# francescofugazzi/3dgsconverter

Measured on NVIDIA H100. Metric: Msplats/s SOR k=16, higher is better.
Workload: dtype f32

## Files before the change

### 3dgsconverter_b200/csrc/gsx_radix.cu

```cuda
#include "../../include/gsx.h"

#include "gsx_common.cuh"
#include "gsx_radix.cuh"

namespace gsx {

#define GSX_FULL 0xffffffffu
constexpr int kRsThreads = 256;
constexpr int kRsPerThread = 16;
constexpr int kRsTile = kRsThreads * kRsPerThread;
constexpr int kRsWarpKeys = 32 * kRsPerThread;
constexpr int kScanBlock = 2048;

__global__ void __launch_bounds__(256) k_scan_block(uint32_t* __restrict__ data, int64_t n,
                                                    uint32_t* __restrict__ sums) {
    const int64_t base = (int64_t)blockIdx.x * kScanBlock + (int64_t)threadIdx.x * 8;
    uint32_t v[8];
    uint32_t tsum = 0;
#pragma unroll
    for (int e = 0; e < 8; ++e) {
        v[e] = base + e < n ? data[base + e] : 0u;
        tsum += v[e];
    }
    uint32_t x = tsum;
// ... 134 lines not shown
        }
        __shared__ uint32_t wtot[8];
        if (lane == 31) wtot[w] = x;
        __syncthreads();
        uint32_t woff = 0;
#pragma unroll
        for (int i = 0; i < 8; ++i)
            if (i < w) woff += wtot[i];
        dstart[threadIdx.x] = woff + x - dcount;
    }
    __syncthreads();
#pragma unroll
    for (int e = 0; e < kRsPerThread; ++e) {
        const int64_t i = wbase + e * 32 + lane;
        if (i < n) {
            const uint32_t d = (uint32_t)(key[e] >> shift) & dmask;
            const uint32_t lp = dstart[d] + wcnt[w][d] + rank[e];
            skeys[lp] = key[e];
            svals[lp] = vals_in[i];
        }
    }
    __syncthreads();
    const int cnt = (int)(n - tbase < kRsTile ? n - tbase : kRsTile);
    for (int j = threadIdx.x; j < cnt; j += kRsThreads) {
        const uint64_t k = skeys[j];
        const uint32_t d = (uint32_t)(k >> shift) & dmask;
        const uint32_t pos = gbase[d] + ((uint32_t)j - dstart[d]);
        keys_out[pos] = k;
        vals_out[pos] = svals[j];
    }
}

constexpr uint32_t kOsAgg = 1u << 30, kOsInc = 1u << 31, kOsVal = (1u << 30) - 1u;
constexpr int kOsMaxPass = 8;
constexpr uint32_t kOsSpinLimit = 1u << 22;

__global__ void __launch_bounds__(256) k_os_hist(const uint64_t* __restrict__ keys, int64_t n, int begin_bit,
                                                  int npass, uint32_t last_mask, uint32_t* __restrict__ ghist) {
    __shared__ uint32_t sh[kOsMaxPass * 256];
    for (int t = threadIdx.x; t < npass * 256; t += 256) sh[t] = 0;
    __syncthreads();
    const int64_t stride = (int64_t)gridDim.x * 256;
    for (int64_t i = (int64_t)blockIdx.x * 256 + threadIdx.x; i < n; i += stride) {
        const uint64_t k = keys[i] >> begin_bit;
        for (int p = 0; p < npass; ++p)
            atomicAdd(&sh[p * 256 + ((uint32_t)(k >> (8 * p)) & (p == npass - 1 ? last_mask : 255u))], 1u);
    }
    __syncthreads();
    for (int t = threadIdx.x; t < npass * 256; t += 256)
        if (sh[t]) atomicAdd(&ghist[t], sh[t]);
}

__global__ void __launch_bounds__(256) k_os_scan(uint32_t* __restrict__ ghist) {
    uint32_t* h = ghist + blockIdx.x * 256;
    const int lane = threadIdx.x & 31, w = threadIdx.x >> 5;
    const uint32_t v = h[threadIdx.x];
    uint32_t x = v;
#pragma unroll
    for (int o = 1; o < 32; o <<= 1) {
        uint32_t y = __shfl_up_sync(GSX_FULL, x, o);
        if (lane >= o) x += y;
    }
    __shared__ uint32_t wt[8];
    if (lane == 31) wt[w] = x;
    __syncthreads();
    uint32_t woff = 0;
#pragma unroll
    for (int i = 0; i < 8; ++i)
        if (i < w) woff += wt[i];
    h[threadIdx.x] = woff + x - v;
}

template <bool PAIRS>
constexpr size_t os_pass_smem() {
    return (size_t)kRsTile * (PAIRS ? 12 : 8) + (size_t)8 * 256 * 4 + 2 * 256 * 4;
}

template <bool PAIRS>
__global__ void __launch_bounds__(kRsThreads, PAIRS ? 3 : 4)
    k_os_pass(const uint64_t* __restrict__ keys_in, const int32_t* __restrict__ vals_in, uint64_t* __restrict__ keys_out,
              int32_t* __restrict__ vals_out, int64_t n, int shift, uint32_t dmask, const uint32_t* __restrict__ gbase_pass,
              uint32_t* lookback, unsigned int* tile_counter) {
// ... 71 lines not shown
        uint32_t woff = 0;
#pragma unroll
        for (int i = 0; i < 8; ++i)
            if (i < w) woff += wtot[i];
        dstart[threadIdx.x] = woff + x - dcount;
    }
    __syncthreads();
#pragma unroll
    for (int e = 0; e < kRsPerThread; ++e) {
        const int64_t i = wbase + e * 32 + lane;
        if (i < n) {
            const uint32_t d = (uint32_t)(key[e] >> shift) & dmask;
            const uint32_t lp = dstart[d] + wcnt[w][d] + ((rank2[e >> 1] >> (16 * (e & 1))) & 0xffffu);
            skeys[lp] = key[e];
            if (PAIRS) svals[lp] = vals_in[i];
        }
    }
    __syncthreads();
    const int cnt = (int)(n - tbase < kRsTile ? n - tbase : kRsTile);
    for (int j = threadIdx.x; j < cnt; j += kRsThreads) {
        const uint64_t k = skeys[j];
        const uint32_t d = (uint32_t)(k >> shift) & dmask;
        const uint32_t pos = gbase[d] + ((uint32_t)j - dstart[d]);
        keys_out[pos] = k;
        if (PAIRS) vals_out[pos] = svals[j];
    }
}

static size_t os_ws_elems(int64_t n) {
    const int64_t ntiles = (n + kRsTile - 1) / kRsTile;
    return (size_t)kOsMaxPass * 256 + 64 + (size_t)kOsMaxPass * 256 * ntiles;
}

template <bool PAIRS>
static int onesweep_sort(uint64_t* keys0, uint64_t* keys1, int32_t* vals0, int32_t* vals1, int64_t n, int begin_bit,
                         int end_bit, uint32_t* ws, uint64_t** keys_sorted, int32_t** vals_sorted, cudaStream_t st) {
    const int64_t ntiles = (n + kRsTile - 1) / kRsTile;
    const int npass = (end_bit - begin_bit + 7) / 8;
    uint32_t* ghist = ws;
    unsigned int* counters = ws + kOsMaxPass * 256;
    uint32_t* lookback = ws + kOsMaxPass * 256 + 64;
    GSX_CUDA_CHECK(cudaMemsetAsync(ws, 0, ((size_t)kOsMaxPass * 256 + 64 + (size_t)npass * 256 * ntiles) * sizeof(uint32_t), st));
    static int hist_blocks = 0;
    if (!hist_blocks) {
        int dev = 0, sms = 132;
        cudaGetDevice(&dev);
        cudaDeviceGetAttribute(&sms, cudaDevAttrMultiProcessorCount, dev);
        hist_blocks = sms * 8;
    }
    int64_t hb = (n + 255) / 256;
    if (hb > hist_blocks) hb = hist_blocks;
    const uint32_t last_mask = digit_mask(begin_bit + 8 * (npass - 1), end_bit);
    k_os_hist<<<(unsigned)hb, 256, 0, st>>>(keys0, n, begin_bit, npass, last_mask, ghist);
    GSX_KERNEL_CHECK();
    k_os_scan<<<npass, 256, 0, st>>>(ghist);
    GSX_KERNEL_CHECK();
    GSX_CUDA_CHECK(cudaFuncSetAttribute(k_os_pass<PAIRS>, cudaFuncAttributeMaxDynamicSharedMemorySize, (int)os_pass_smem<PAIRS>()));
    uint64_t *kin = keys0, *kout = keys1;
    int32_t *vin = vals0, *vout = vals1;
    for (int p = 0; p < npass; ++p) {
        k_os_pass<PAIRS><<<(unsigned)ntiles, kRsThreads, os_pass_smem<PAIRS>(), st>>>(
            kin, vin, kout, vout, n, begin_bit + 8 * p, p == npass - 1 ? last_mask : 255u, ghist + p * 256,
            lookback + (size_t)p * 256 * ntiles, counters + p);
        GSX_KERNEL_CHECK();
        uint64_t* tk = kin;
        kin = kout;
        kout = tk;
        int32_t* tv = vin;
        vin = vout;
        vout = tv;
    }
    *keys_sorted = kin;
    if (vals_sorted) *vals_sorted = vin;
    return GSX_OK;
}

size_t radix_ws_bytes(int64_t n) {
    if (n < 1) n = 1;
    int64_t ntiles = (n + kRsTile - 1) / kRsTile;
    size_t hist = (size_t)256 * ntiles;
    size_t three_kernel = hist + scan_ws_elems((int64_t)hist) + 256;
    size_t onesweep = os_ws_elems(n);
    return (three_kernel > onesweep ? three_kernel : onesweep) * sizeof(uint32_t);
}

int radix_sort_pairs(uint64_t* keys0, uint64_t* keys1, int32_t* vals0, int32_t* vals1, int64_t n, int begin_bit,
                     int end_bit, void* ws, size_t ws_bytes, uint64_t** keys_sorted, int32_t** vals_sorted,
                     cudaStream_t st) {
    GSX_NVTX("gsx::radix_sort_pairs");
    GSX_REQUIRE(n >= 1 && n < 4294967296ll, GSX_ERR_ARG, "radix: n out of range");
    GSX_REQUIRE(ws_bytes >= radix_ws_bytes(n), GSX_ERR_WORKSPACE, "radix: workspace too small");
    GSX_REQUIRE(begin_bit >= 0 && end_bit <= 64 && begin_bit < end_bit, GSX_ERR_ARG, "radix: bad bit range");
    if (n < (1ll << 30))
        return onesweep_sort<true>(keys0, keys1, vals0, vals1, n, begin_bit, end_bit, (uint32_t*)ws, keys_sorted,
                                   vals_sorted, st);
    const int64_t ntiles = (n + kRsTile - 1) / kRsTile;
    uint32_t* hist = (uint32_t*)ws;
    uint32_t* scan_ws = hist + (size_t)256 * ntiles;
    GSX_CUDA_CHECK(cudaFuncSetAttribute(k_rs_scatter, cudaFuncAttributeMaxDynamicSharedMemorySize, (int)kRsScatterSmem));
    uint64_t *kin = keys0, *kout = keys1;
    int32_t *vin = vals0, *vout = vals1;
    for (int shift = begin_bit; shift < end_bit; shift += 8) {
        const uint32_t dmask = digit_mask(shift, end_bit);
        k_rs_hist<<<(unsigned)ntiles, kRsThreads, 0, st>>>(kin, n, shift, dmask, ntiles, hist);
        GSX_KERNEL_CHECK();
        int rc = exclusive_scan_u32(hist, (int64_t)256 * ntiles, scan_ws, st);
        if (rc) return rc;
        k_rs_scatter<<<(unsigned)ntiles, kRsThreads, kRsScatterSmem, st>>>(kin, vin, kout, vout, n, shift, dmask, ntiles,
                                                                          hist);
        GSX_KERNEL_CHECK();
        uint64_t* tk = kin;
        kin = kout;
        kout = tk;
        int32_t* tv = vin;
        vin = vout;
        vout = tv;
    }
    *keys_sorted = kin;
    *vals_sorted = vin;
    return GSX_OK;
}

int radix_sort_keys(uint64_t* keys0, uint64_t* keys1, int64_t n, int begin_bit, int end_bit, void* ws, size_t ws_bytes,
                    uint64_t** keys_sorted, cudaStream_t st) {
    GSX_NVTX("gsx::radix_sort_keys");
    GSX_REQUIRE(n >= 1 && n < (1ll << 30), GSX_ERR_ARG, "radix: n out of range");
    GSX_REQUIRE(ws_bytes >= radix_ws_bytes(n), GSX_ERR_WORKSPACE, "radix: workspace too small");
    GSX_REQUIRE(begin_bit >= 0 && end_bit <= 64 && begin_bit < end_bit, GSX_ERR_ARG, "radix: bad bit range");
    return onesweep_sort<false>(keys0, keys1, nullptr, nullptr, n, begin_bit, end_bit, (uint32_t*)ws, keys_sorted, nullptr,
                                st);
}

}

using namespace gsx;

extern "C" {

int64_t gsx_sort_pairs_workspace_bytes(int64_t n) {
    if (n < 1) n = 1;
    return (int64_t)(align_up((size_t)n * 8, 256) + align_up((size_t)n * 4, 256) + radix_ws_bytes(n) + 1024);
}

int gsx_sort_pairs(uint64_t* keys_dev, int32_t* vals_dev, int64_t n, int32_t begin_bit, int32_t end_bit, void* ws,
                   int64_t ws_bytes, void* stream) {
    cudaStream_t st = (cudaStream_t)stream;
    if (n == 0) return GSX_OK;
    GSX_REQUIRE(ws_bytes >= gsx_sort_pairs_workspace_bytes(n), GSX_ERR_WORKSPACE, "sort: workspace too small");
    Carver c(ws, (size_t)ws_bytes);
    uint64_t* k1 = c.take<uint64_t>((size_t)n);
    int32_t* v1 = c.take<int32_t>((size_t)n);
    char* rws = c.take<char>(radix_ws_bytes(n));
    uint64_t* ks = nullptr;
    int32_t* vs = nullptr;
    int rc = vals_dev ? radix_sort_pairs(keys_dev, k1, vals_dev, v1, n, begin_bit, end_bit, rws, radix_ws_bytes(n), &ks,
                                         &vs, st)
                      : radix_sort_keys(keys_dev, k1, n, begin_bit, end_bit, rws, radix_ws_bytes(n), &ks, st);
    if (rc) return rc;
    if (ks != keys_dev) {
        GSX_CUDA_CHECK(cudaMemcpyAsync(keys_dev, ks, (size_t)n * 8, cudaMemcpyDeviceToDevice, st));
        if (vals_dev) GSX_CUDA_CHECK(cudaMemcpyAsync(vals_dev, vs, (size_t)n * 4, cudaMemcpyDeviceToDevice, st));
    }
    return GSX_OK;
}

// ... 2 lines not shown
```

### 3dgsconverter_b200/csrc/gsx_radix.cuh

```cuda
#pragma once
#include "gsx_common.cuh"
namespace gsx {
size_t radix_ws_bytes(int64_t n);
size_t scan_workspace_bytes(int64_t n);
int exclusive_scan_u32_ws(uint32_t* data, int64_t n, uint32_t* ws, cudaStream_t st);
int radix_sort_pairs(uint64_t* keys0, uint64_t* keys1, int32_t* vals0, int32_t* vals1, int64_t n, int begin_bit,
                     int end_bit, void* ws, size_t ws_bytes, uint64_t** keys_sorted, int32_t** vals_sorted,
                     cudaStream_t st);
int radix_sort_keys(uint64_t* keys0, uint64_t* keys1, int64_t n, int begin_bit, int end_bit, void* ws, size_t ws_bytes,
                    uint64_t** keys_sorted, cudaStream_t st);
}
```

### 3dgsconverter_b200/csrc/gsx_sor.cu

```cuda
#include "../../include/gsx.h"

#include "gsx_bits.cuh"
#include "gsx_common.cuh"
#include "gsx_sor.cuh"

#include "gsx_radix.cuh"
#include <math.h>

namespace gsx {

#define GSX_D2LIM_BITS 0x60ad78ebu
#define GSX_FULL 0xffffffffu

constexpr int kCellCodeBits = 15;
constexpr float kCellCodeScale = (float)(1 << (kCellCodeBits / 3));
constexpr float kCellCodeMax = kCellCodeScale - 1.f;
constexpr int kSmallBucket = 64;
constexpr int kQueryBatch = 16;
constexpr int kMergeThreshold = 9;
constexpr int kKnnMinBlocks = 8;
constexpr int kFlatSupers = 8;
const char* sor_build_info() {
    return "knn=r03a;epi_smem=1;first_sort=1;query_batch=16;minblocks=8;merge_threshold=9;small_bucket=64;"
           "flat_supers=8;knn16=0;tma=0;i32=1;cell_order=hilbert15";
// ... 160 lines not shown

struct PackFmt {
    int idx_bits, mort_bits, bucket_bits;
    __host__ __device__ int key_shift() const { return idx_bits + mort_bits; }
    __host__ __device__ uint64_t idx_mask() const { return (1ull << idx_bits) - 1ull; }
    __host__ __device__ int sort_begin() const { return idx_bits; }
    __host__ __device__ int sort_end() const { return idx_bits + mort_bits + bucket_bits; }
};

static int bits_for(int64_t n) {
    int b = 1;
    while (((int64_t)1 << b) < n) ++b;
    return b;
}

static PackFmt pack_fmt(int64_t n_items, int64_t n_buckets) {
    PackFmt f;
    f.idx_bits = bits_for(n_items);
    f.bucket_bits = bits_for(n_buckets);
    int avail = 64 - f.idx_bits - f.bucket_bits;
    if (avail > kCellCodeBits) avail = kCellCodeBits;
    f.mort_bits = avail < 0 ? 0 : avail - avail % 3;
    return f;
}

__device__ __forceinline__ uint64_t pack_word(uint64_t key , uint64_t bucket_sub,
                                              int64_t idx, PackFmt f) {
    const uint64_t bucket = (key >> kCellCodeBits) - bucket_sub;
    const uint64_t mort = (key & ((1ull << kCellCodeBits) - 1ull)) >> (kCellCodeBits - f.mort_bits);
    return (((bucket << f.mort_bits) | mort) << f.idx_bits) | (uint64_t)idx;
}

__global__ void __launch_bounds__(256) k_sor_keys(const float* __restrict__ xyz, int64_t n, float bx, float by,
                                                  float bz, float cell, uint64_t M64, PackFmt f,
                                                  uint64_t* __restrict__ keys) {
    int64_t i = (int64_t)blockIdx.x * blockDim.x + threadIdx.x;
    if (i >= n) return;
    keys[i] = pack_word(bucket_key(xyz[3 * i], xyz[3 * i + 1], xyz[3 * i + 2], bx, by, bz, cell, n, M64), 0, i, f);
}

template <bool GATHER>
__device__ __forceinline__ void
    sor_finish_tile(const int64_t tile, const float* __restrict__ xyz, const uint64_t* __restrict__ keys, PackFmt fmt,
                    float4* __restrict__ spos, int64_t n, float bx, float by, float bz, float cell, uint64_t M64,
                    int2* __restrict__ tab_se, uint32_t* __restrict__ startbits, uint32_t* __restrict__ cellbits,
                    float4* __restrict__ caabb, float4* __restrict__ saabb) {
    const int64_t j = tile * 1024 + threadIdx.x;
    const int lane = lane_id();
    float lo[3] = {INFINITY, INFINITY, INFINITY}, hi[3] = {-INFINITY, -INFINITY, -INFINITY};
    uint32_t h = 0xffffffffu;
    auto hash_at = [&](int64_t t) -> uint32_t {
        if (GATHER) return (uint32_t)(keys[t] >> fmt.key_shift());
        const float4 q = spos[t];
        return bucket_of(q.x, q.y, q.z, bx, by, bz, cell, n, M64);
    };
    int gcx = 0x7fffffff, gcy = 0, gcz = 0;
    if (j < n) {
        float x, y, z;
        if (GATHER) {
            const uint64_t word = keys[j];
            const int32_t idx = (int32_t)(word & fmt.idx_mask());
            x = xyz[3 * (int64_t)idx], y = xyz[3 * (int64_t)idx + 1], z = xyz[3 * (int64_t)idx + 2];
            spos[j] = make_float4(x, y, z, __int_as_float(idx));
            h = (uint32_t)(word >> fmt.key_shift());
        } else {
            const float4 p = spos[j];
            x = p.x, y = p.y, z = p.z;
            h = bucket_of(x, y, z, bx, by, bz, cell, n, M64);
        }
        gcx = (int)floorf(__fdiv_rn(__fsub_rn(x, bx), cell));
        gcy = (int)floorf(__fdiv_rn(__fsub_rn(y, by), cell));
// ... 328 lines not shown
        float lo[3], hi[3];
        bucket_box_partial(spos, caabb, s, end, lane, lo, hi);
#pragma unroll
        for (int a = 0; a < 3; ++a) {
            lo[a] = ord_to_float(__reduce_min_sync(GSX_FULL, float_to_ord(lo[a])));
            hi[a] = ord_to_float(__reduce_max_sync(GSX_FULL, float_to_ord(hi[a])));
        }
        if (lane == 0) {
            tab_se[hb].y = (int)end;
            tab_box[2 * (size_t)hb] = make_float4(lo[0], lo[1], lo[2], 0.f);
            tab_box[2 * (size_t)hb + 1] = make_float4(hi[0], hi[1], hi[2], 0.f);
        }
    }
    }
    }
}

template <bool GATHER>
static int sor_finish(const float* xyz, int64_t n, const float* bmin, float cell, SorWs& w, PackFmt fmt, cudaStream_t st) {
    const uint64_t M64 = 0xFFFFFFFFFFFFFFFFull / (uint64_t)n;
    GSX_CUDA_CHECK(cudaMemsetAsync(w.tab_se, 0, (size_t)n * sizeof(int2), st));
    k_sor_finish<GATHER><<<(int)((n + 1023) / 1024), 1024, 0, st>>>(xyz, w.keys_sorted, fmt, w.spos, n, bmin[0],
                                                                    bmin[1], bmin[2], cell, M64, w.tab_se, w.startbits,
                                                                    w.cellbits, w.caabb, w.saabb);
    GSX_KERNEL_CHECK();
    k_sor_bucket_boxes<<<(int)((n + 255) / 256), 256, 0, st>>>(w.startbits, w.spos, w.caabb, w.tab_se, n, bmin[0],
                                                               bmin[1], bmin[2], cell, M64, w.tab_box);
    GSX_KERNEL_CHECK();
    return GSX_OK;
}

int sor_build(const float* xyz, int64_t n, const float* bmin, float cell, SorWs& w, cudaStream_t st) {
    GSX_NVTX("gsx::sor_build");
    int blocks = (int)((n + 255) / 256);
    const PackFmt fmt = pack_fmt(n, n);
    k_sor_keys<<<blocks, 256, 0, st>>>(xyz, n, bmin[0], bmin[1], bmin[2], cell, 0xFFFFFFFFFFFFFFFFull / (uint64_t)n,
                                       fmt, w.keys0);
    GSX_KERNEL_CHECK();
    {
        int rc = radix_sort_keys(w.keys0, w.keys1, n, fmt.sort_begin(), fmt.sort_end(), w.sort_ws, w.sort_ws_bytes,
                                 &w.keys_sorted, st);
        if (rc) return rc;
    }
    return sor_finish<true>(xyz, n, bmin, cell, w, fmt, st);
}


__global__ void __launch_bounds__(256) k_sor_owner_keys(const float* __restrict__ xyz, int64_t n, int64_t n_global,
                                                        int world, float bx, float by, float bz, float cell,
                                                        uint64_t M64, int idx_bits, uint64_t* __restrict__ keys) {
    int64_t i = (int64_t)blockIdx.x * blockDim.x + threadIdx.x;
    if (i >= n) return;
    uint64_t h = bucket_key(xyz[3 * i], xyz[3 * i + 1], xyz[3 * i + 2], bx, by, bz, cell, n_global, M64) >> kCellCodeBits;
    keys[i] = (((h * (uint64_t)world) / (uint64_t)n_global) << idx_bits) | (uint64_t)i;
}

__global__ void __launch_bounds__(256) k_sor_gather_slab(const float* __restrict__ xyz,
                                                         const uint64_t* __restrict__ words, uint64_t idx_mask, int64_t n,
                                                         int64_t idx_base, float4* __restrict__ pos4) {
    int64_t j = (int64_t)blockIdx.x * blockDim.x + threadIdx.x;
    if (j >= n) return;
    int32_t idx = (int32_t)(words[j] & idx_mask);
    pos4[j] = make_float4(xyz[3 * (int64_t)idx], xyz[3 * (int64_t)idx + 1], xyz[3 * (int64_t)idx + 2],
                          __int_as_float((int)(idx_base + idx)));
}

__global__ void k_sor_owner_counts(const uint64_t* __restrict__ owners_sorted, int idx_bits, int64_t n, int world,
                                   long long* __restrict__ cuts) {
    int o = threadIdx.x;
    if (o > world) return;
    int64_t lo = 0, hi = n;
    while (lo < hi) {
        int64_t mid = (lo + hi) >> 1;
        if ((owners_sorted[mid] >> idx_bits) < (uint64_t)o) lo = mid + 1; else hi = mid;
// ... 462 lines not shown
                   const float* bmin, float cell,
                   float* final_means, unsigned long long* stats, cudaStream_t st) {
    GSX_NVTX("gsx::sor_mean_dists(k_sor_knn)");
    int64_t n = w.n;
    GSX_REQUIRE(k >= 1, GSX_ERR_ARG, "sor: k must be >= 1 (got %d)", k);
    GSX_REQUIRE(hash_mode == 0 || hash_mode == 1, GSX_ERR_ARG, "sor: bad hash_mode %d", hash_mode);
    GSX_REQUIRE(q_begin >= 0 && q_end <= n && q_begin <= q_end, GSX_ERR_ARG, "sor: bad query range");
    GSX_REQUIRE(q_stride >= 1 && q_phase >= 0 && q_phase < q_stride, GSX_ERR_ARG, "sor: bad query stride/phase");
    int K = k < 50 ? k : 50;
    if (stats) GSX_CUDA_CHECK(cudaMemsetAsync(w.stats, 0, kCntCount * sizeof(unsigned long long), st));
    if (q_end == q_begin) return GSX_OK;
    if (!(cell > 1e-8f)) {
        GSX_REQUIRE(q_begin == 0 && q_end == n, GSX_ERR_UNSUPPORTED, "sor: degenerate cell with a query range");
        k_fill_f32<<<(int)((n + 255) / 256), 256, 0, st>>>(final_means, n, 0.f);
        GSX_KERNEL_CHECK();
        return GSX_OK;
    }
    GSX_CUDA_CHECK(cudaMemsetAsync(w.counters, 0, sizeof(unsigned int), st));
    uint64_t M = 0xFFFFFFFFFFFFFFFFull / (uint64_t)n + 1ull;
    int64_t nq = (q_end - q_begin + q_stride - 1) / q_stride + kQueryBatch;
    int64_t want = (nq + (int64_t)kQueryBatch * 8 - 1) / ((int64_t)kQueryBatch * 8);
    int rc;
    if (K <= 16)
        rc = launch_knn<1, 17>(w, q_begin, q_end, q_stride, q_phase, K, hash_mode, bmin, cell, final_means, stats, M, want, st);
    else if (K <= 32)
        rc = launch_knn<1, 33>(w, q_begin, q_end, q_stride, q_phase, K, hash_mode, bmin, cell, final_means, stats, M, want, st);
    else
        rc = launch_knn<2, 0>(w, q_begin, q_end, q_stride, q_phase, K, hash_mode, bmin, cell, final_means, stats, M, want, st);
    if (rc) return rc;
    GSX_KERNEL_CHECK();
    return GSX_OK;
}

static int carve_grid_checked(void* ws, int64_t ws_bytes, int64_t n, SorWs& w) {
    GSX_REQUIRE(n >= 1 && n < 2147483584ll, GSX_ERR_ARG, "sor: n=%lld out of range [1, 2^31-64)", (long long)n);
    GSX_REQUIRE(ws != nullptr, GSX_ERR_WORKSPACE, "sor: null workspace");
    w = sor_carve(ws, ws_bytes, n, sor_sort_ws_bytes(n));
    GSX_REQUIRE(w.grid_ok, GSX_ERR_WORKSPACE, "sor: grid workspace too small (%lld < %zu)", (long long)ws_bytes,
                w.grid_total);
    return GSX_OK;
}

static int carve_checked(void* ws, int64_t ws_bytes, int64_t n, SorWs& w) {
    GSX_REQUIRE(n >= 1 && n < 2147483584ll, GSX_ERR_ARG, "sor: n=%lld out of range [1, 2^31-64)", (long long)n);
    GSX_REQUIRE(ws != nullptr, GSX_ERR_WORKSPACE, "sor: null workspace");
    w = sor_carve(ws, ws_bytes, n, sor_sort_ws_bytes(n));
    GSX_REQUIRE(w.ok, GSX_ERR_WORKSPACE, "sor: workspace too small (%lld < %zu)", (long long)ws_bytes, w.total);
    return GSX_OK;
}

}

using namespace gsx;

extern "C" {

int64_t gsx_sor_workspace_bytes(int64_t n) {
    if (n < 1) n = 1;
    SorWs w = sor_carve(nullptr, 0, n, sor_sort_ws_bytes(n));
    return (int64_t)w.total + 1024;
}

int64_t gsx_sor_grid_workspace_bytes(int64_t n) {
    if (n < 1) n = 1;
    SorWs w = sor_carve(nullptr, 0, n, sor_sort_ws_bytes(n));
    return (int64_t)w.grid_total;
// ... 2 lines not shown

int gsx_sor_minmax(const float* xyz_dev, int64_t n, float* minmax_dev, void* ws, int64_t ws_bytes, void* stream) {
    GSX_REQUIRE(n >= 1, GSX_ERR_ARG, "sor: minmax of an empty cloud");
    GSX_REQUIRE(ws != nullptr && ws_bytes >= 6 * 1024 * (int64_t)sizeof(float), GSX_ERR_WORKSPACE,
                "sor: minmax needs 24 KiB of scratch");
    return sor_minmax(xyz_dev, n, minmax_dev, (float*)ws, (cudaStream_t)stream);
}

float gsx_sor_cell_size(const float* mm, int64_t n) {
    float ex = mm[3] - mm[0], ey = mm[4] - mm[1], ez = mm[5] - mm[2];
    float vol = (ex * ey) * ez;
    double cell;
    if (vol <= 0.0f || vol != vol) {
        if (vol != vol) {
            cell = NAN;
        } else {
            double avg = 1.0 / (double)n;
            if (!(avg > 1e-8)) avg = 1e-8;
            cell = pow(avg * 32.0, 1.0 / 3.0);
        }
    } else {
        float avgf = vol / (float)n;
        if ((double)avgf > 1e-8) {
            float cv = avgf * 32.0f;
            cell = (double)powf(cv, (float)(1.0 / 3.0));
        } else {
            cell = pow(1e-8 * 32.0, 1.0 / 3.0);
        }
    }
    if (!(cell > 1e-4)) cell = 1e-4;
    return (float)cell;
}

int gsx_sor_build(const float* xyz_dev, int64_t n, const float* bmin_host, float cell, void* ws, int64_t ws_bytes,
                  void* stream) {
    SorWs w;
    int rc = carve_checked(ws, ws_bytes, n, w);
    if (rc) return rc;
    GSX_REQUIRE(cell > 0.f, GSX_ERR_ARG, "sor: cell size must be > 0");
    return sor_build(xyz_dev, n, bmin_host, cell, w, (cudaStream_t)stream);
}

int gsx_sor_dist_local_run(const float* xyz_local_dev, int64_t n_local, int64_t idx_base, int64_t n_global,
                           int32_t world, const float* bmin_host, float cell, float* pos4_out_dev,
                           int64_t* cuts_dev, void* ws, int64_t ws_bytes, void* stream) {
    SorWs w;
    int rc = carve_checked(ws, ws_bytes, n_local > 0 ? n_local : 1, w);
    if (rc) return rc;
    GSX_REQUIRE(n_global >= n_local && n_global >= 1 && n_global < 2147483584ll, GSX_ERR_ARG, "sor: bad n_global");
    return sor_dist_local_run(xyz_local_dev, n_local, idx_base, n_global, world, bmin_host, cell,
                              (float4*)pos4_out_dev, (long long*)cuts_dev, w, (cudaStream_t)stream);
}

int gsx_sor_dist_merge(const float* pos4_dev, int64_t m, int64_t n_global, int64_t bucket_lo, int64_t bucket_hi,
                       const float* bmin_host, float cell, float* pos4_sorted_dev, uint8_t* flags_sorted_dev, void* ws,
                       int64_t ws_bytes, void* stream) {
    if (m == 0) return GSX_OK;
    SorWs w;
    int rc = carve_checked(ws, ws_bytes, m, w);
    if (rc) return rc;
    return sor_dist_merge((const float4*)pos4_dev, m, n_global, bucket_lo, bucket_hi, bmin_host, cell,
                          (float4*)pos4_sorted_dev, flags_sorted_dev, w, (cudaStream_t)stream);
}

int64_t gsx_sor_spos_offset(int64_t n) {
    if (n < 1) return -1;
// ... 24 lines not shown
                               const float* bmin_host, float cell, void* ws, int64_t ws_bytes, float* final_means_dev,
                               unsigned long long* stats_dev, void* stream) {
    SorWs w;
    int rc = carve_grid_checked(ws, ws_bytes, n, w);
    if (rc) return rc;
    return sor_mean_dists(w, 0, n, stride, phase, k, hash_mode, bmin_host, cell, final_means_dev, stats_dev,
                          (cudaStream_t)stream);
}

int gsx_sor_mean_dists(int64_t n, int32_t k, int32_t hash_mode, const float* bmin_host, float cell, void* ws,
                       int64_t ws_bytes, float* final_means_dev, unsigned long long* stats_dev, void* stream) {
    return gsx_sor_mean_dists_range(n, 0, n, k, hash_mode, bmin_host, cell, ws, ws_bytes, final_means_dev, stats_dev,
                                    stream);
}

int gsx_sor_query_counters(int64_t n, void* ws, int64_t ws_bytes, unsigned long long* out8_host, void* stream) {
    SorWs w;
    int rc = carve_grid_checked(ws, ws_bytes, n, w);
    if (rc) return rc;
    GSX_REQUIRE(out8_host != nullptr, GSX_ERR_ARG, "sor: null counter buffer");
    GSX_CUDA_CHECK(cudaMemcpyAsync(out8_host, w.stats, 8 * sizeof(unsigned long long), cudaMemcpyDeviceToHost,
                                   (cudaStream_t)stream));
    GSX_CUDA_CHECK(cudaStreamSynchronize((cudaStream_t)stream));
    return GSX_OK;
}

int gsx_sor_filter_device(const float* xyz_dev, int64_t n, int32_t k, float threshold_factor, int32_t hash_mode,
                          uint8_t* mask_dev, float* means_dev, void* ws, int64_t ws_bytes, void* stream) {
    cudaStream_t st = (cudaStream_t)stream;
    SorWs w;
    int rc = carve_checked(ws, ws_bytes, n, w);
    if (rc) return rc;
    GSX_REQUIRE(k >= 1, GSX_ERR_ARG, "sor: k must be >= 1 (got %d)", k);
    if ((rc = sor_minmax(xyz_dev, n, w.minmax, w.partial, st))) return rc;
    float mm[6];
    GSX_CUDA_CHECK(cudaMemcpyAsync(mm, w.minmax, sizeof(mm), cudaMemcpyDeviceToHost, st));
    GSX_CUDA_CHECK(cudaStreamSynchronize(st));
    float cell = gsx_sor_cell_size(mm, n);
    GSX_REQUIRE(cell == cell, GSX_ERR_ARG, "sor: non-finite coordinates");
    if ((rc = sor_build(xyz_dev, n, mm, cell, w, st))) return rc;
    float* means = means_dev ? means_dev : reinterpret_cast<float*>(w.keys0);
    if ((rc = sor_mean_dists(w, 0, n, 1, 0, k, hash_mode, mm, cell, means, nullptr, st))) return rc;
    if ((rc = mean_std_f32(means, n, w.meanstd, w.ms_ws, w.ms_bytes, st))) return rc;
    return threshold_mask(means, n, w.meanstd, threshold_factor, mask_dev, st);
}

}
```

### 3dgsconverter_b200/gsx/sor.py

```python
from __future__ import annotations

import ctypes as C
from dataclasses import dataclass

import numpy as np
import torch

from . import _abi
from ._abi import lib, check, HASH_MODES, _ptr, _stream


def default_hash_mode() -> str:
    import os
    return os.environ.get("GSX_SOR_HASH", "i32wrap")


def _check_xyz(xyz: torch.Tensor):
    if xyz.dim() != 2 or xyz.shape[1] != 3:
        raise ValueError("Requires 3D data")
    if not xyz.is_cuda or xyz.dtype != torch.float32 or not xyz.is_contiguous():
        raise ValueError("xyz must be a contiguous float32 CUDA tensor [N,3]")


@dataclass
class SorGrid:
    n: int
    ws: torch.Tensor
    bmin: np.ndarray
    cell: float


def workspace(n: int, device) -> torch.Tensor:
    nbytes = lib.gsx_sor_workspace_bytes(n)
    if nbytes <= 0:
        raise _abi.GsxError("gsx_sor_workspace_bytes failed")
    return torch.empty(nbytes, dtype=torch.uint8, device=device)


def build_grid(xyz: torch.Tensor, ws: torch.Tensor | None = None, cell_scale: float = 1.0) -> SorGrid:
    _check_xyz(xyz)
    n = xyz.shape[0]
    if ws is None:
        ws = workspace(n, xyz.device)
    mm_dev = torch.empty(8, dtype=torch.float32, device=xyz.device)
    check(lib.gsx_sor_minmax(_ptr(xyz), n, _ptr(mm_dev), _ptr(ws), ws.numel(), _stream()), "gsx_sor_minmax")
    mm = mm_dev[:6].cpu().numpy()
    cell = float(lib.gsx_sor_cell_size(mm.ctypes.data_as(C.POINTER(C.c_float)), n))
    if cell != cell:
        raise _abi.GsxError("sor: non-finite coordinates")
    if cell_scale != 1.0:
        cell = float(np.float32(cell * cell_scale))
    bmin = mm[:3].copy()
    check(lib.gsx_sor_build(_ptr(xyz), n, bmin.ctypes.data_as(C.POINTER(C.c_float)), cell, _ptr(ws), ws.numel(),
                            _stream()), "gsx_sor_build")
    return SorGrid(n, ws, bmin, cell)


QUERY_COUNTERS = ("inserts", "merges_first", "merges_full", "probe_visits", "super_visits", "chunk_groups",
                  "chunk_visits", "scan_steps")


def _stats_dict(grid: SorGrid, stats: torch.Tensor) -> dict:
    v = stats.cpu().numpy()
    c = (C.c_ulonglong * 8)()
    check(lib.gsx_sor_query_counters(grid.n, _ptr(grid.ws), grid.ws.numel(), C.cast(c, C.c_void_p), _stream()),
          "gsx_sor_query_counters")
    return dict(visits=int(v[0]), scanned=int(v[1]), box_tests=int(v[2]), queries=int(v[3]),
                **{name: int(c[i]) for i, name in enumerate(QUERY_COUNTERS)})


def mean_dists(grid: SorGrid, k: int, hash_mode: str | None = None, out: torch.Tensor | None = None,
               want_stats: bool = False, q_range: tuple[int, int] | None = None):
    mode = HASH_MODES[hash_mode or default_hash_mode()]
    dev = grid.ws.device
    if out is None:
        out = torch.empty(grid.n, dtype=torch.float32, device=dev)
    stats = torch.zeros(4, dtype=torch.int64, device=dev) if want_stats else None
    qb, qe = q_range if q_range is not None else (0, grid.n)
    check(lib.gsx_sor_mean_dists_range(grid.n, qb, qe, int(k), mode, grid.bmin.ctypes.data_as(C.POINTER(C.c_float)),
                                       grid.cell, _ptr(grid.ws), grid.ws.numel(), _ptr(out), _ptr(stats), _stream()),
          "gsx_sor_mean_dists")
    if want_stats:
        return out, _stats_dict(grid, stats)
    return out


def mean_dists_strided(grid: SorGrid, k: int, hash_mode: str | None, out: torch.Tensor, stride: int, phase: int,
# ... 93 lines not shown
```

### include/gsx.h

```cpp
#ifndef GSX_H
#define GSX_H
#include <stdint.h>

#ifdef __cplusplus
extern "C" {
#endif

#define GSX_HASH_I32WRAP 0
#define GSX_HASH_I64 1

const char* gsx_last_error(void);
int gsx_version(void);
const char* gsx_build_info(void);
int gsx_device_sm_count(void);
long long gsx_kernel_launches(void);


int64_t gsx_sor_workspace_bytes(int64_t n);
int64_t gsx_sor_grid_workspace_bytes(int64_t n);

int gsx_sor_minmax(const float* xyz_dev, int64_t n, float* minmax_dev, void* ws, int64_t ws_bytes, void* stream);

float gsx_sor_cell_size(const float* minmax_host, int64_t n);

int gsx_sor_build(const float* xyz_dev, int64_t n, const float* bmin_host, float cell, void* ws, int64_t ws_bytes,
                  void* stream);

int gsx_sor_dist_local_run(const float* xyz_local_dev, int64_t n_local, int64_t idx_base, int64_t n_global,
                           int32_t world, const float* bmin_host, float cell, float* pos4_out_dev,
                           int64_t* cuts_dev, void* ws, int64_t ws_bytes, void* stream);
int gsx_sor_dist_merge(const float* pos4_dev, int64_t m, int64_t n_global, int64_t bucket_lo, int64_t bucket_hi,
                       const float* bmin_host, float cell, float* pos4_sorted_dev,
                       uint8_t* flags_sorted_dev , void* ws, int64_t ws_bytes, void* stream);
int64_t gsx_sor_spos_offset(int64_t n);
int gsx_sor_build_from_sorted(const float* spos4_dev, const uint8_t* flags_dev , int64_t n,
                              const float* bmin_host, float cell, void* ws, int64_t ws_bytes, void* stream);

int gsx_sor_mean_dists(int64_t n, int32_t k, int32_t hash_mode, const float* bmin_host, float cell, void* ws,
                       int64_t ws_bytes, float* final_means_dev, unsigned long long* stats_dev, void* stream);

int gsx_sor_mean_dists_range(int64_t n, int64_t q_begin, int64_t q_end, int32_t k, int32_t hash_mode,
                             const float* bmin_host, float cell, void* ws, int64_t ws_bytes, float* final_means_dev,
                             unsigned long long* stats_dev, void* stream);

int gsx_sor_mean_dists_strided(int64_t n, int32_t stride, int32_t phase, int32_t k, int32_t hash_mode,
                               const float* bmin_host, float cell, void* ws, int64_t ws_bytes, float* final_means_dev,
                               unsigned long long* stats_dev, void* stream);

int gsx_sor_query_counters(int64_t n, void* ws, int64_t ws_bytes, unsigned long long* out8_host, void* stream);

int64_t gsx_sort_pairs_workspace_bytes(int64_t n);
int gsx_sort_pairs(uint64_t* keys_dev, int32_t* vals_dev, int64_t n, int32_t begin_bit, int32_t end_bit, void* ws,
                   int64_t ws_bytes, void* stream);

int64_t gsx_mean_std_workspace_bytes(int64_t n);
int gsx_mean_std_f32(const float* a_dev, int64_t n, float* out_dev, void* ws, int64_t ws_bytes, void* stream);

int64_t gsx_pairwise_slots(int64_t n);
int gsx_pairwise_leaves_dist(const float* a_local_dev, int64_t base, int64_t n_local, int64_t n_global, int32_t sq,
// ... 211 lines not shown
```

Measured before the change: 1288.

## Fuse radix digit histogram into SOR key generation and merge grid build host calls

The key-generation kernel now becomes a grid-stride kernel that also accumulates the onesweep radix digit histograms in shared memory, so the sort no longer runs a separate histogram pass that re-reads all keys. The radix sort is split into clear, counted-histogram and pass phases to allow this. The Python grid build also replaces several separate host calls (minmax, copy to host, cell size, build) with a single native entry point. The cost is a key kernel limited to a capped grid, with shared-memory atomics inside it.

```diff
diff --git a/3dgsconverter_b200/csrc/gsx_radix.cu b/3dgsconverter_b200/csrc/gsx_radix.cu
--- a/3dgsconverter_b200/csrc/gsx_radix.cu
+++ b/3dgsconverter_b200/csrc/gsx_radix.cu
@@ -190,22 +190,17 @@
 }
 
 constexpr uint32_t kOsAgg = 1u << 30, kOsInc = 1u << 31, kOsVal = (1u << 30) - 1u;
-constexpr int kOsMaxPass = 8;
 constexpr uint32_t kOsSpinLimit = 1u << 22;
 
-__global__ void __launch_bounds__(256) k_os_hist(const uint64_t* __restrict__ keys, int64_t n, int begin_bit,
-                                                  int npass, uint32_t last_mask, uint32_t* __restrict__ ghist) {
+__global__ void __launch_bounds__(256) k_os_hist(const uint64_t* __restrict__ keys, int64_t n, OsDigits dg,
+                                                  uint32_t* __restrict__ ghist) {
     __shared__ uint32_t sh[kOsMaxPass * 256];
-    for (int t = threadIdx.x; t < npass * 256; t += 256) sh[t] = 0;
+    for (int t = threadIdx.x; t < dg.npass * 256; t += 256) sh[t] = 0;
     __syncthreads();
     const int64_t stride = (int64_t)gridDim.x * 256;
-    for (int64_t i = (int64_t)blockIdx.x * 256 + threadIdx.x; i < n; i += stride) {
-        const uint64_t k = keys[i] >> begin_bit;
-        for (int p = 0; p < npass; ++p)
-            atomicAdd(&sh[p * 256 + ((uint32_t)(k >> (8 * p)) & (p == npass - 1 ? last_mask : 255u))], 1u);
-    }
-    __syncthreads();
-    for (int t = threadIdx.x; t < npass * 256; t += 256)
+    for (int64_t i = (int64_t)blockIdx.x * 256 + threadIdx.x; i < n; i += stride) os_count(sh, keys[i], dg);
+    __syncthreads();
+    for (int t = threadIdx.x; t < dg.npass * 256; t += 256)
         if (sh[t]) atomicAdd(&ghist[t], sh[t]);
 }
 
@@ -343,27 +338,32 @@
     return (size_t)kOsMaxPass * 256 + 64 + (size_t)kOsMaxPass * 256 * ntiles;
 }
 
+OsDigits os_digits(int begin_bit, int end_bit) {
+    OsDigits d;
+    d.begin_bit = begin_bit;
+    d.npass = (end_bit - begin_bit + 7) / 8;
+    d.last_mask = digit_mask(begin_bit + 8 * (d.npass - 1), end_bit);
+    return d;
+}
+
+uint32_t* radix_counted_hist(void* ws) { return (uint32_t*)ws; }
+
+static int os_clear(int64_t n, int npass, uint32_t* ws, cudaStream_t st) {
+    const int64_t ntiles = (n + kRsTile - 1) / kRsTile;
+    GSX_CUDA_CHECK(cudaMemsetAsync(ws, 0, ((size_t)kOsMaxPass * 256 + 64 + (size_t)npass * 256 * ntiles) * sizeof(uint32_t), st));
+    return GSX_OK;
+}
+
 template <bool PAIRS>
-static int onesweep_sort(uint64_t* keys0, uint64_t* keys1, int32_t* vals0, int32_t* vals1, int64_t n, int begin_bit,
-                         int end_bit, uint32_t* ws, uint64_t** keys_sorted, int32_t** vals_sorted, cudaStream_t st) {
+static int os_passes(uint64_t* keys0, uint64_t* keys1, int32_t* vals0, int32_t* vals1, int64_t n, int begin_bit,
+                     int end_bit, uint32_t* ws, uint64_t** keys_sorted, int32_t** vals_sorted, cudaStream_t st) {
     const int64_t ntiles = (n + kRsTile - 1) / kRsTile;
-    const int npass = (end_bit - begin_bit + 7) / 8;
+    const OsDigits dg = os_digits(begin_bit, end_bit);
+    const int npass = dg.npass;
+    const uint32_t last_mask = dg.last_mask;
     uint32_t* ghist = ws;
     unsigned int* counters = ws + kOsMaxPass * 256;
     uint32_t* lookback = ws + kOsMaxPass * 256 + 64;
-    GSX_CUDA_CHECK(cudaMemsetAsync(ws, 0, ((size_t)kOsMaxPass * 256 + 64 + (size_t)npass * 256 * ntiles) * sizeof(uint32_t), st));
-    static int hist_blocks = 0;
-    if (!hist_blocks) {
-        int dev = 0, sms = 132;
-        cudaGetDevice(&dev);
-        cudaDeviceGetAttribute(&sms, cudaDevAttrMultiProcessorCount, dev);
-        hist_blocks = sms * 8;
-    }
-    int64_t hb = (n + 255) / 256;
-    if (hb > hist_blocks) hb = hist_blocks;
-    const uint32_t last_mask = digit_mask(begin_bit + 8 * (npass - 1), end_bit);
-    k_os_hist<<<(unsigned)hb, 256, 0, st>>>(keys0, n, begin_bit, npass, last_mask, ghist);
-    GSX_KERNEL_CHECK();
     k_os_scan<<<npass, 256, 0, st>>>(ghist);
     GSX_KERNEL_CHECK();
     GSX_CUDA_CHECK(cudaFuncSetAttribute(k_os_pass<PAIRS>, cudaFuncAttributeMaxDynamicSharedMemorySize, (int)os_pass_smem<PAIRS>()));
@@ -384,6 +384,19 @@
     *keys_sorted = kin;
     if (vals_sorted) *vals_sorted = vin;
     return GSX_OK;
+}
+
+template <bool PAIRS>
+static int onesweep_sort(uint64_t* keys0, uint64_t* keys1, int32_t* vals0, int32_t* vals1, int64_t n, int begin_bit,
+                         int end_bit, uint32_t* ws, uint64_t** keys_sorted, int32_t** vals_sorted, cudaStream_t st) {
+    const OsDigits dg = os_digits(begin_bit, end_bit);
+    int rc = os_clear(n, dg.npass, ws, st);
+    if (rc) return rc;
+    int64_t hb = (n + 255) / 256;
+    if (hb > sm_count() * 8) hb = sm_count() * 8;
+    k_os_hist<<<(unsigned)hb, 256, 0, st>>>(keys0, n, dg, ws);
+    GSX_KERNEL_CHECK();
+    return os_passes<PAIRS>(keys0, keys1, vals0, vals1, n, begin_bit, end_bit, ws, keys_sorted, vals_sorted, st);
 }
 
 size_t radix_ws_bytes(int64_t n) {
@@ -442,6 +455,23 @@
                                 st);
 }
 
+int radix_counted_clear(int64_t n, int begin_bit, int end_bit, void* ws, size_t ws_bytes, cudaStream_t st) {
+    GSX_REQUIRE(n >= 1 && n < (1ll << 30), GSX_ERR_ARG, "radix: n out of range");
+    GSX_REQUIRE(ws_bytes >= radix_ws_bytes(n), GSX_ERR_WORKSPACE, "radix: workspace too small");
+    GSX_REQUIRE(begin_bit >= 0 && end_bit <= 64 && begin_bit < end_bit, GSX_ERR_ARG, "radix: bad bit range");
+    return os_clear(n, os_digits(begin_bit, end_bit).npass, (uint32_t*)ws, st);
+}
+
+int radix_sort_counted(uint64_t* keys0, uint64_t* keys1, int64_t n, int begin_bit, int end_bit, void* ws,
+                       size_t ws_bytes, uint64_t** keys_sorted, cudaStream_t st) {
+    GSX_NVTX("gsx::radix_sort_counted");
+    GSX_REQUIRE(n >= 1 && n < (1ll << 30), GSX_ERR_ARG, "radix: n out of range");
+    GSX_REQUIRE(ws_bytes >= radix_ws_bytes(n), GSX_ERR_WORKSPACE, "radix: workspace too small");
+    GSX_REQUIRE(begin_bit >= 0 && end_bit <= 64 && begin_bit < end_bit, GSX_ERR_ARG, "radix: bad bit range");
+    return os_passes<false>(keys0, keys1, nullptr, nullptr, n, begin_bit, end_bit, (uint32_t*)ws, keys_sorted, nullptr,
+                            st);
+}
+
 }
 
 using namespace gsx;
diff --git a/3dgsconverter_b200/csrc/gsx_radix.cuh b/3dgsconverter_b200/csrc/gsx_radix.cuh
--- a/3dgsconverter_b200/csrc/gsx_radix.cuh
+++ b/3dgsconverter_b200/csrc/gsx_radix.cuh
@@ -9,4 +9,21 @@
                      cudaStream_t st);
 int radix_sort_keys(uint64_t* keys0, uint64_t* keys1, int64_t n, int begin_bit, int end_bit, void* ws, size_t ws_bytes,
                     uint64_t** keys_sorted, cudaStream_t st);
+
+constexpr int kOsMaxPass = 8;
+struct OsDigits {
+    int begin_bit, npass;
+    uint32_t last_mask;
+};
+OsDigits os_digits(int begin_bit, int end_bit);
+int radix_counted_clear(int64_t n, int begin_bit, int end_bit, void* ws, size_t ws_bytes, cudaStream_t st);
+uint32_t* radix_counted_hist(void* ws);
+int radix_sort_counted(uint64_t* keys0, uint64_t* keys1, int64_t n, int begin_bit, int end_bit, void* ws,
+                       size_t ws_bytes, uint64_t** keys_sorted, cudaStream_t st);
+
+__device__ __forceinline__ void os_count(uint32_t* sh, uint64_t key, OsDigits d) {
+    const uint64_t k = key >> d.begin_bit;
+    for (int p = 0; p < d.npass; ++p)
+        atomicAdd(&sh[p * 256 + ((uint32_t)(k >> (8 * p)) & (p == d.npass - 1 ? d.last_mask : 255u))], 1u);
 }
+}
diff --git a/3dgsconverter_b200/csrc/gsx_sor.cu b/3dgsconverter_b200/csrc/gsx_sor.cu
--- a/3dgsconverter_b200/csrc/gsx_sor.cu
+++ b/3dgsconverter_b200/csrc/gsx_sor.cu
@@ -216,11 +216,21 @@
 }
 
 __global__ void __launch_bounds__(256) k_sor_keys(const float* __restrict__ xyz, int64_t n, float bx, float by,
-                                                  float bz, float cell, uint64_t M64, PackFmt f,
-                                                  uint64_t* __restrict__ keys) {
-    int64_t i = (int64_t)blockIdx.x * blockDim.x + threadIdx.x;
-    if (i >= n) return;
-    keys[i] = pack_word(bucket_key(xyz[3 * i], xyz[3 * i + 1], xyz[3 * i + 2], bx, by, bz, cell, n, M64), 0, i, f);
+                                                  float bz, float cell, uint64_t M64, PackFmt f, OsDigits dg,
+                                                  uint64_t* __restrict__ keys, uint32_t* __restrict__ ghist) {
+    __shared__ uint32_t sh[kOsMaxPass * 256];
+    for (int t = threadIdx.x; t < dg.npass * 256; t += 256) sh[t] = 0;
+    __syncthreads();
+    const int64_t stride = (int64_t)gridDim.x * 256;
+    for (int64_t i = (int64_t)blockIdx.x * 256 + threadIdx.x; i < n; i += stride) {
+        const uint64_t w = pack_word(bucket_key(xyz[3 * i], xyz[3 * i + 1], xyz[3 * i + 2], bx, by, bz, cell, n, M64), 0,
+                                     i, f);
+        keys[i] = w;
+        os_count(sh, w, dg);
+    }
+    __syncthreads();
+    for (int t = threadIdx.x; t < dg.npass * 256; t += 256)
+        if (sh[t]) atomicAdd(&ghist[t], sh[t]);
 }
 
 template <bool GATHER>
@@ -615,14 +625,21 @@
 
 int sor_build(const float* xyz, int64_t n, const float* bmin, float cell, SorWs& w, cudaStream_t st) {
     GSX_NVTX("gsx::sor_build");
-    int blocks = (int)((n + 255) / 256);
     const PackFmt fmt = pack_fmt(n, n);
-    k_sor_keys<<<blocks, 256, 0, st>>>(xyz, n, bmin[0], bmin[1], bmin[2], cell, 0xFFFFFFFFFFFFFFFFull / (uint64_t)n,
-                                       fmt, w.keys0);
-    GSX_KERNEL_CHECK();
     {
-        int rc = radix_sort_keys(w.keys0, w.keys1, n, fmt.sort_begin(), fmt.sort_end(), w.sort_ws, w.sort_ws_bytes,
-                                 &w.keys_sorted, st);
+        int rc = radix_counted_clear(n, fmt.sort_begin(), fmt.sort_end(), w.sort_ws, w.sort_ws_bytes, st);
+        if (rc) return rc;
+    }
+    int64_t blocks = (n + 255) / 256;
+    if (blocks > sm_count() * 8) blocks = sm_count() * 8;
+    k_sor_keys<<<(unsigned)blocks, 256, 0, st>>>(xyz, n, bmin[0], bmin[1], bmin[2], cell,
+                                                 0xFFFFFFFFFFFFFFFFull / (uint64_t)n, fmt,
+                                                 os_digits(fmt.sort_begin(), fmt.sort_end()), w.keys0,
+                                                 radix_counted_hist(w.sort_ws));
+    GSX_KERNEL_CHECK();
+    {
+        int rc = radix_sort_counted(w.keys0, w.keys1, n, fmt.sort_begin(), fmt.sort_end(), w.sort_ws, w.sort_ws_bytes,
+                                    &w.keys_sorted, st);
         if (rc) return rc;
     }
     return sor_finish<true>(xyz, n, bmin, cell, w, fmt, st);
@@ -1151,6 +1168,23 @@
     return GSX_OK;
 }
 
+}
+extern "C" float gsx_sor_cell_size(const float* mm, int64_t n);
+namespace gsx {
+
+static int sor_build_grid(const float* xyz, int64_t n, double cell_scale, float (&mm)[6], float& cell, SorWs& w,
+                          cudaStream_t st) {
+    int rc = sor_minmax(xyz, n, w.minmax, w.partial, st);
+    if (rc) return rc;
+    GSX_CUDA_CHECK(cudaMemcpyAsync(mm, w.minmax, sizeof(mm), cudaMemcpyDeviceToHost, st));
+    GSX_CUDA_CHECK(cudaStreamSynchronize(st));
+    cell = gsx_sor_cell_size(mm, n);
+    GSX_REQUIRE(cell == cell, GSX_ERR_ARG, "sor: non-finite coordinates");
+    if (cell_scale != 1.0) cell = (float)((double)cell * cell_scale);
+    GSX_REQUIRE(cell > 0.f, GSX_ERR_ARG, "sor: cell size must be > 0");
+    return sor_build(xyz, n, mm, cell, w, st);
+}
+
 static int carve_grid_checked(void* ws, int64_t ws_bytes, int64_t n, SorWs& w) {
     GSX_REQUIRE(n >= 1 && n < 2147483584ll, GSX_ERR_ARG, "sor: n=%lld out of range [1, 2^31-64)", (long long)n);
     GSX_REQUIRE(ws != nullptr, GSX_ERR_WORKSPACE, "sor: null workspace");
@@ -1219,6 +1253,18 @@
     return (float)cell;
 }
 
+int gsx_sor_build_grid(const float* xyz_dev, int64_t n, double cell_scale, float* bmin_cell_host, void* ws,
+                       int64_t ws_bytes, void* stream) {
+    SorWs w;
+    int rc = carve_checked(ws, ws_bytes, n, w);
+    if (rc) return rc;
+    GSX_REQUIRE(bmin_cell_host != nullptr, GSX_ERR_ARG, "sor: null bmin/cell output");
+    float mm[6], cell;
+    if ((rc = sor_build_grid(xyz_dev, n, cell_scale, mm, cell, w, (cudaStream_t)stream))) return rc;
+    bmin_cell_host[0] = mm[0], bmin_cell_host[1] = mm[1], bmin_cell_host[2] = mm[2], bmin_cell_host[3] = cell;
+    return GSX_OK;
+}
+
 int gsx_sor_build(const float* xyz_dev, int64_t n, const float* bmin_host, float cell, void* ws, int64_t ws_bytes,
                   void* stream) {
     SorWs w;
@@ -1309,13 +1355,8 @@
     int rc = carve_checked(ws, ws_bytes, n, w);
     if (rc) return rc;
     GSX_REQUIRE(k >= 1, GSX_ERR_ARG, "sor: k must be >= 1 (got %d)", k);
-    if ((rc = sor_minmax(xyz_dev, n, w.minmax, w.partial, st))) return rc;
-    float mm[6];
-    GSX_CUDA_CHECK(cudaMemcpyAsync(mm, w.minmax, sizeof(mm), cudaMemcpyDeviceToHost, st));
-    GSX_CUDA_CHECK(cudaStreamSynchronize(st));
-    float cell = gsx_sor_cell_size(mm, n);
-    GSX_REQUIRE(cell == cell, GSX_ERR_ARG, "sor: non-finite coordinates");
-    if ((rc = sor_build(xyz_dev, n, mm, cell, w, st))) return rc;
+    float mm[6], cell;
+    if ((rc = sor_build_grid(xyz_dev, n, 1.0, mm, cell, w, st))) return rc;
     float* means = means_dev ? means_dev : reinterpret_cast<float*>(w.keys0);
     if ((rc = sor_mean_dists(w, 0, n, 1, 0, k, hash_mode, mm, cell, means, nullptr, st))) return rc;
     if ((rc = mean_std_f32(means, n, w.meanstd, w.ms_ws, w.ms_bytes, st))) return rc;
diff --git a/3dgsconverter_b200/gsx/sor.py b/3dgsconverter_b200/gsx/sor.py
--- a/3dgsconverter_b200/gsx/sor.py
+++ b/3dgsconverter_b200/gsx/sor.py
@@ -42,17 +42,10 @@
     n = xyz.shape[0]
     if ws is None:
         ws = workspace(n, xyz.device)
-    mm_dev = torch.empty(8, dtype=torch.float32, device=xyz.device)
-    check(lib.gsx_sor_minmax(_ptr(xyz), n, _ptr(mm_dev), _ptr(ws), ws.numel(), _stream()), "gsx_sor_minmax")
-    mm = mm_dev[:6].cpu().numpy()
-    cell = float(lib.gsx_sor_cell_size(mm.ctypes.data_as(C.POINTER(C.c_float)), n))
-    if cell != cell:
-        raise _abi.GsxError("sor: non-finite coordinates")
-    if cell_scale != 1.0:
-        cell = float(np.float32(cell * cell_scale))
-    bmin = mm[:3].copy()
-    check(lib.gsx_sor_build(_ptr(xyz), n, bmin.ctypes.data_as(C.POINTER(C.c_float)), cell, _ptr(ws), ws.numel(),
-                            _stream()), "gsx_sor_build")
+    out = np.empty(4, dtype=np.float32)
+    check(lib.gsx_sor_build_grid(_ptr(xyz), n, float(cell_scale), out.ctypes.data_as(C.POINTER(C.c_float)), _ptr(ws),
+                                 ws.numel(), _stream()), "gsx_sor_build_grid")
+    bmin, cell = out[:3].copy(), float(out[3])
     return SorGrid(n, ws, bmin, cell)
 
 
diff --git a/include/gsx.h b/include/gsx.h
--- a/include/gsx.h
+++ b/include/gsx.h
@@ -25,6 +25,9 @@
 
 int gsx_sor_build(const float* xyz_dev, int64_t n, const float* bmin_host, float cell, void* ws, int64_t ws_bytes,
                   void* stream);
+
+int gsx_sor_build_grid(const float* xyz_dev, int64_t n, double cell_scale, float* bmin_cell_host, void* ws,
+                       int64_t ws_bytes, void* stream);
 
 int gsx_sor_dist_local_run(const float* xyz_local_dev, int64_t n_local, int64_t idx_base, int64_t n_global,
                            int32_t world, const float* bmin_host, float cell, float* pos4_out_dev,
```

New measurement: 1307 (median of 6 runs). +1.5%, better.
